# lukehollis/three-mlagents

Measured on NVIDIA B200. Metric: env_steps_per_sec, higher is better.
Workload: dtype f32+f64

## Files before the change

profiles/rollout_sass.py:

```python
from __future__ import annotations

import argparse
import os
import re
import subprocess
import sys
import tempfile

ROOT = os.path.dirname(os.path.dirname(os.path.abspath(__file__)))
FLAGS = ["-gencode", "arch=compute_100a,code=sm_100a", "-lineinfo", "-O3", "-std=c++17", "--expt-relaxed-constexpr"]
INS = re.compile(r"^\s+/\*([0-9a-f]{4,})\*/\s+(.*?)\s*;")


def _compile(tree, tmp):
    csrc = os.path.join(tree, "three-mlagents_b200", "csrc")
    cubin = os.path.join(tmp, "env_kernels.cubin")
    nvcc = os.path.join(os.environ.get("CUDA_HOME", "/usr/local/cuda"), "bin", "nvcc")
    r = subprocess.run([nvcc, *FLAGS, "-I", os.path.join(tree, "include"), "-Xptxas", "-v", "-cubin", "-o", cubin,
                        os.path.join(csrc, "env_kernels.cu")], capture_output=True, text=True)
    if r.returncode != 0:
        raise SystemExit(r.stdout + r.stderr)
    return cubin, r.stdout + r.stderr


def _ptxas(log, mangled):
    lines = log.splitlines()
    for n, line in enumerate(lines):
        if f"'{mangled}'" in line and "Compiling entry" in line:
            text = " ".join(lines[n + 1:n + 4])
            num = lambda pat: int(re.search(pat, text).group(1))
            return {"registers": num(r"Used (\d+) registers"), "stack_bytes": num(r"(\d+) bytes stack frame"),
                    "spill_store_bytes": num(r"(\d+) bytes spill stores"), "spill_load_bytes": num(r"(\d+) bytes spill loads")}
    raise SystemExit(f"{mangled}: no ptxas report")


def _sass(cubin, mangled):
    out = subprocess.run(["cuobjdump", "-sass", "-fun", mangled, cubin], capture_output=True, text=True, check=True).stdout
    return [(int(m.group(1), 16), m.group(2)) for m in map(INS.match, out.splitlines()) if m]


def _branch(ins):
    m = re.match(r"(@!?U?P\w+\s+)?BRA(\.U)?\s+(!?U?P\w+,\s*)?(0x[0-9a-f]+)", ins)
    if not m:
        return None
    return int(m.group(4), 16), bool(m.group(1) or m.group(3))


def _loops(code):
    loops = []
    for addr, ins in code:
        b = _branch(ins)
        if b and b[0] <= addr:
            loops.append((b[0], addr))
    return [(h, e) for h, e in loops if not any(h <= h2 and e2 <= e and (h2, e2) != (h, e) for h2, e2 in loops)]


def _shortest(code, head, end):
    body = [(a, ins) for a, ins in code if head <= a <= end]
    index = {a: n for n, (a, _) in enumerate(body)}
    inf = (1 << 30, 0, 0)
    best = [inf] * (len(body) + 1)
    best[0] = (0, 0, 0)
    for n, (a, ins) in enumerate(body):
        if best[n] == inf:
            continue
        c, br, st = best[n]
        here = (c + 1, br + (_branch(ins) is not None), st + ("STG" in ins and ".U8" in ins))
        if a == end:
            best[len(body)] = min(best[len(body)], here)
            continue
        b = _branch(ins)
        nxt = []
        if b is None or b[1]:
            if not re.match(r"(EXIT|RET)", ins):
                nxt.append(n + 1)
        if b and head < b[0] <= end and b[0] in index:
            nxt.append(index[b[0]])
        for m in nxt:
            best[m] = min(best[m], here)
    return best[len(body)]


def main():
    ap = argparse.ArgumentParser()
    ap.add_argument("--tree", default=ROOT, help="repository tree whose env_kernels.cu is compiled")
    ap.add_argument("--tasks", default="Ball3D,GridWorld,Push")
    args = ap.parse_args()
    with tempfile.TemporaryDirectory(prefix="rollout_sass_") as tmp:
        cubin, log = _compile(os.path.abspath(args.tree), tmp)
        for task in args.tasks.split(","):
            name = f"{task}Task"
            mangled = f"_Z19rollout_fast_kernelI{len(name)}{name}Ev7EnvPtrsjmmmiP6float4PiPfPh"
            res = _ptxas(log, mangled)
            code = _sass(cubin, mangled)
            print(f"rollout_fast_kernel<{name}>: {res['registers']} registers, stack {res['stack_bytes']} B, "
                  f"spills {res['spill_store_bytes']} B stored / {res['spill_load_bytes']} B loaded, {len(code) * 16} B of code")
            for head, end in _loops(code):
                ins, br, steps = _shortest(code, head, end)
                if not steps:
                    continue
                per = f", per step {ins / steps:.1f} instructions and {br / steps:.1f} branches"
                print(f"    loop 0x{head:x}-0x{end:x}: {end + 16 - head} B, shortest path {ins} instructions, "
                      f"{br} branches, {steps} steps{per}")


if __name__ == "__main__":
    sys.exit(main())
```

three-mlagents_b200/csrc/env_handle.cuh:

```cuda
#pragma once
#include "common.cuh"

struct tmla_env {
    int task;
    int64_t n;
    uint64_t seed, env_id_base, step_count;
    int device;
    void *buf[4];
    int *err_flag;
    void *d_stage, *h_stage;
    size_t stage_bytes;
    cudaStream_t own_stream;
    int32_t *d_ndone;
    int64_t rec_hint;
    cudaStream_t dev_stream;
    bool dev_dirty;
    cudaEvent_t dev_evt;
    int act_u8;
    void *shadow[4];
    int pend_seq;
    float2 *ep_log;
    int32_t ep_log_cap;
    int32_t *ep_log_count;
    void *rollout_plan;
    void (*rollout_plan_free)(void *);
};

struct DeviceGuard {
    int prev = -1;
    bool switched = false;
    explicit DeviceGuard(int dev) {
        if (cudaGetDevice(&prev) == cudaSuccess && prev != dev) switched = cudaSetDevice(dev) == cudaSuccess;
    }
    ~DeviceGuard() { if (switched) cudaSetDevice(prev); }
};
static inline void mark_device_path(tmla_env *h, cudaStream_t st) { h->dev_stream = st; h->dev_dirty = true; }
```

three-mlagents_b200/csrc/env_kernels.cu:

```cuda
#include <stdarg.h>
#include <stdlib.h>
#include <string.h>
#include <new>
#include <type_traits>
#if defined(__x86_64__)
#include <immintrin.h>
#endif
#include "envs.cuh"
#include "env_handle.cuh"

static int order_after_device_path(tmla_env *h) {
    if (!h->dev_dirty) return TMLA_OK;
    h->dev_dirty = false;
    cudaStreamCaptureStatus cap = cudaStreamCaptureStatusNone;
    if (cudaStreamIsCapturing(h->dev_stream, &cap) != cudaSuccess || cap != cudaStreamCaptureStatusNone ||
        cudaEventRecord(h->dev_evt, h->dev_stream) != cudaSuccess) {
        cudaGetLastError();
        TMLA_CUDA(cudaDeviceSynchronize());
        return TMLA_OK;
    }
    TMLA_CUDA(cudaStreamWaitEvent(h->own_stream, h->dev_evt, 0));
    return TMLA_OK;
}

struct EnvPtrs { void *buf[4]; };

static constexpr int kBlock = 128;

template <int D, int BLOCK, bool STREAMING>
__device__ __forceinline__ void block_store_obs(const float *s_obs, float *dst, int valid_envs) {
    const int total = valid_envs * D;
    if ((reinterpret_cast<uintptr_t>(dst) & 15u) == 0) {
        const int nvec = total >> 2;
        const float4 *s4 = reinterpret_cast<const float4 *>(s_obs);
        float4 *d4 = reinterpret_cast<float4 *>(dst);
        for (int v = threadIdx.x; v < nvec; v += BLOCK) {
            if (STREAMING) st_stream_f4(d4 + v, s4[v]);
            else d4[v] = s4[v];
        }
        for (int e = (nvec << 2) + threadIdx.x; e < total; e += BLOCK) dst[e] = s_obs[e];
    } else {
        for (int e = threadIdx.x; e < total; e += BLOCK) dst[e] = s_obs[e];
    }
}

template <int D>
__device__ __forceinline__ void thread_store_obs(const float *o, float *dst) {
#pragma unroll
    for (int j = 0; j < D; ++j) dst[j] = o[j];
}

template <class Task>
__global__ void __launch_bounds__(kBlock) reset_kernel(EnvPtrs p, int64_t n, uint64_t seed, uint64_t env_base,
                                                       uint64_t k, uint32_t tag, float *obs) {
    __shared__ __align__(16) float s_obs[kBlock * Task::D];
    const int64_t i0 = (int64_t)blockIdx.x * kBlock, i = i0 + threadIdx.x;
    if (i < n) {
        typename Task::State s;
        Task::reset(s, seed, env_base + (uint64_t)i, k, tag);
        Task::store(p.buf, i, s);
        float o[Task::D];
        Task::observe(s, o);
#pragma unroll
        for (int j = 0; j < Task::D; ++j) s_obs[threadIdx.x * Task::D + j] = o[j];
    }
    __syncthreads();
    if (obs) block_store_obs<Task::D, kBlock, false>(s_obs, obs + i0 * Task::D, (int)min((int64_t)kBlock, n - i0));
}

template <class Task>
__global__ void get_state_kernel(EnvPtrs p, int64_t n, typename Task::Wire *aos) {
    const int64_t i = (int64_t)blockIdx.x * blockDim.x + threadIdx.x;
    if (i < n) aos[i] = Task::to_wire(Task::load(p.buf, i));
}
template <class Task>
__global__ void set_state_kernel(EnvPtrs p, int64_t n, const typename Task::Wire *aos) {
    const int64_t i = (int64_t)blockIdx.x * blockDim.x + threadIdx.x;
    if (i < n) Task::store(p.buf, i, Task::from_wire(aos[i]));
}

template <class Task>
__global__ void __launch_bounds__(kBlock)
step_kernel(EnvPtrs p, int64_t n, uint64_t seed, uint64_t env_base, uint64_t step_index,
            const int32_t *__restrict__ actions, float *__restrict__ obs, float *__restrict__ reward,
            uint8_t *__restrict__ done, uint8_t *__restrict__ truncated, float *__restrict__ terminal_obs,
            float *__restrict__ ep_return, int32_t *__restrict__ ep_length, int32_t *n_done, int *err_flag,
            float *__restrict__ compact, int32_t *__restrict__ host_flags, int host_seq, int act_u8,
            const int32_t *ready, int32_t *dev_ready, int chunk_ctas, EnvPtrs shadow) {
    constexpr int D = Task::D;
    __shared__ __align__(16) float s_obs[kBlock * D];
    __shared__ __align__(16) float s_rew[kBlock];
    __shared__ __align__(16) uint8_t s_flag[2 * kBlock];
    const int64_t i0 = (int64_t)blockIdx.x * kBlock, i = i0 + threadIdx.x;
    if (ready) {
// ... 106 lines not shown
template <class Task>
__global__ void __launch_bounds__(kRollBlock)
rollout_random_kernel(EnvPtrs p, int64_t n, uint64_t seed, uint64_t env_base, uint64_t step0, int T,
                      float *__restrict__ obs_buf, int32_t *__restrict__ act_buf, float *__restrict__ rew_buf,
                      uint8_t *__restrict__ done_buf) {
    constexpr int D = Task::D, BLOCK = kRollBlock;
    constexpr bool STAGED = (D != 4);
    constexpr int NVEC = BLOCK * D / 4;
    __shared__ __align__(16) float s_obs[STAGED ? 2 * BLOCK * D : 4];
    const int64_t i0 = (int64_t)blockIdx.x * BLOCK, i = i0 + threadIdx.x;
    const bool active = i < n;
    const int valid = (int)min((int64_t)BLOCK, n - i0);
    const uint64_t env_id = env_base + (uint64_t)i;
    const int64_t row_floats = n * D;
    const bool vec_ok = obs_buf && valid == BLOCK && ((reinterpret_cast<uintptr_t>(obs_buf + i0 * D) & 15u) == 0) &&
                        ((row_floats & 3) == 0);
    const typename Task::Consts cst = Task::load_consts();
    typename Task::State s;
    TmlaActionStream as;
    if (active) {
        s = Task::load(p.buf, i);
        as.seek(seed, env_id, step0, Task::A);
    }
    float *orow = obs_buf ? obs_buf + i0 * D : nullptr;
    int64_t off = i;
    for (int t = 0; t < T; ++t) {
        const uint64_t k = step0 + (uint64_t)t;
        float *stage = STAGED ? s_obs + (t & 1) * BLOCK * D : s_obs;
        if (active) {
            float o[D];
            Task::observe(s, o);
            if (STAGED) stage_obs<D>(stage, o);
            else if (obs_buf) {
                float *dst = obs_buf + off * 4;
                if ((reinterpret_cast<uintptr_t>(obs_buf) & 15u) == 0) st_stream_f4(reinterpret_cast<float4 *>(dst), make_float4(o[0], o[1], o[2], o[3]));
                else { dst[0] = o[0]; dst[1] = o[1]; dst[2] = o[2]; dst[3] = o[3]; }
            }
            const int a = as.next(seed, env_id, step0, (uint32_t)t, Task::A);
            float r; bool term, trunc;
            Task::step(cst, s, a, r, term, trunc);
            s.ep_ret = __fadd_rn(s.ep_ret, r);
            const bool d = term || trunc;
            if (act_buf) __stcs(act_buf + off, a);
            if (rew_buf) __stcs(rew_buf + off, r);
            if (done_buf) __stcs(done_buf + off, (uint8_t)(d ? 1 : 0));
            if (d) Task::reset(s, seed, env_id, k + 1, TMLA_TAG_RESET);
        }
        if (STAGED) {
            __syncthreads();
            if (vec_ok) {
                const float4 *s4 = reinterpret_cast<const float4 *>(stage);
                float4 *d4 = reinterpret_cast<float4 *>(orow);
#pragma unroll
                for (int v = 0; v < (NVEC + BLOCK - 1) / BLOCK; ++v) {
                    const int e = v * BLOCK + threadIdx.x;
                    if ((v + 1) * BLOCK <= NVEC || e < NVEC) st_stream_f4(d4 + e, s4[e]);
                }
            } else if (obs_buf) {
                block_store_obs<D, BLOCK, true>(stage, orow, valid);
            }
            if (orow) orow += row_floats;
        }
        off += n;
    }
    if (active) Task::store(p.buf, i, s);
}

#ifndef TMLA_SPARE_EVERY
#define TMLA_SPARE_EVERY 64
#endif
static constexpr int kSpareEvery = TMLA_SPARE_EVERY;
#ifndef TMLA_ROLLOUT_UNROLL
#define TMLA_ROLLOUT_UNROLL 2
#endif
static constexpr int kRollUnroll = TMLA_ROLLOUT_UNROLL;
static_assert(kSpareEvery % 16 == 0 && ((kSpareEvery / 16) & (kSpareEvery / 16 - 1)) == 0, "a power-of-two number of action blocks");
static_assert(16 % kRollUnroll == 0, "the unrolled step loop covers whole action blocks");

template <class Task>
__device__ __noinline__ typename Task::Spare draw_spare(uint64_t seed, uint64_t env_id, uint32_t episode) {
    return Task::draw(seed, env_id, episode, TMLA_TAG_RESET);
}

template <class Task>
__global__ void __launch_bounds__(kRollBlock)
rollout_fast_kernel(EnvPtrs p, uint32_t n, uint64_t seed, uint64_t env_base, uint64_t step0, int T,
                    float4 *__restrict__ obs4, int32_t *__restrict__ act_buf, float *__restrict__ rew_buf,
                    uint8_t *__restrict__ done_buf) {
    constexpr int D = Task::D, BLOCK = kRollBlock, NVEC = BLOCK * D / 4;
    static_assert(Task::A <= 16, "actions are packed as 4-bit digits");
    constexpr bool DIRECT = (D == 6);
    constexpr bool STAGED = (D != 4) && !DIRECT;
    static_assert((BLOCK * D) % 4 == 0, "block rows must be whole float4s");
    __shared__ __align__(16) float s_stage[STAGED ? 2 * BLOCK * D : 4];
    const uint32_t tid = threadIdx.x, i = blockIdx.x * BLOCK + tid;
    const uint64_t env_id = env_base + (uint64_t)i;
    const typename Task::Consts cst = Task::load_consts();
    typename Task::State s = Task::load(p.buf, i);
    float *orow = reinterpret_cast<float *>(obs4) + (size_t)i * D;
    float4 *vrow = obs4 + blockIdx.x * NVEC + tid;
    int32_t *arow = act_buf + i;
    float *rrow = rew_buf + i;
    uint8_t *drow = done_buf + i;
    const uint32_t rowfloats = n * D;
    uint32_t sb = 0;
    [[maybe_unused]] typename Task::Spare sp;
    [[maybe_unused]] bool have_spare = false;
    auto step = [&](uint64_t digits, uint32_t j, uint64_t kb) {
        float o[D];
        Task::observe(s, o);
        if constexpr (STAGED) {
            if constexpr (D % 2 == 0) {
                float2 *s2 = reinterpret_cast<float2 *>(s_stage + sb + tid * D);
#pragma unroll
                for (int q = 0; q < D / 2; ++q) s2[q] = make_float2(o[2 * q], o[2 * q + 1]);
            } else {
#pragma unroll
                for (int q = 0; q < D; ++q) s_stage[sb + tid * D + q] = o[q];
            }
        } else if constexpr (DIRECT) {
            float2 *d2 = reinterpret_cast<float2 *>(orow);
#pragma unroll
            for (int q = 0; q < D / 2; ++q) __stcs(d2 + q, make_float2(o[2 * q], o[2 * q + 1]));
        } else {
            st_stream_f4(reinterpret_cast<float4 *>(orow), make_float4(o[0], o[1], o[2], o[3]));
        }
        const int a = (int)((uint32_t)(digits >> (4 * j)) & 15u);
        float r; bool term, trunc;
        Task::step(cst, s, a, r, term, trunc);
        s.ep_ret = __fadd_rn(s.ep_ret, r);
        const bool d = term || trunc;
        __stcs(arow, a);
        __stcs(rrow, r);
        __stcs(drow, (uint8_t)(d ? 1 : 0));
        if (d) {
            if constexpr (Task::HAS_SPARE) {
                const uint32_t e = Task::next_episode(s);
                if (!have_spare) sp = draw_spare<Task>(seed, env_id, e);
                Task::begin_episode(s, sp, e);
                have_spare = false;
            } else {
                Task::reset(s, seed, env_id, kb + j + 1, TMLA_TAG_RESET);
            }
        }
        if constexpr (STAGED) {
            if constexpr (BLOCK == 32) __syncwarp(); else __syncthreads();
            const float4 *s4 = reinterpret_cast<const float4 *>(s_stage + sb);
#pragma unroll
            for (int v = 0; v < (NVEC + BLOCK - 1) / BLOCK; ++v) {
                const int e = v * BLOCK + tid;
                if ((v + 1) * BLOCK <= NVEC || e < NVEC) st_stream_f4(vrow + v * BLOCK, s4[e]);
            }
            sb ^= BLOCK * D;
            vrow += rowfloats / 4;
        } else {
            orow += rowfloats;
        }
        arow += n; rrow += n; drow += n;
    };
    uint64_t kb = step0 & ~(uint64_t)15;
    uint32_t j = (uint32_t)step0 & 15u;
    uint32_t left = (uint32_t)T;
    for (uint32_t nb = 0; left != 0; ++nb, kb += 16, j = 0) {
        const uint64_t digits = TmlaActionStream::block_digits(seed, env_id, kb >> 4, Task::A);
        if constexpr (Task::HAS_SPARE) {
            if ((nb & (kSpareEvery / 16 - 1)) == 0 && !have_spare) {
                sp = Task::draw(seed, env_id, Task::next_episode(s), TMLA_TAG_RESET);
                have_spare = true;
            }
        }
        if (j == 0 && left >= 16) {
#pragma unroll kRollUnroll
            for (uint32_t q = 0; q < 16; ++q) step(digits, q, kb);
            left -= 16;
        } else {
            const uint32_t je = min(16u, j + left);
            left -= je - j;
#pragma unroll 1
            for (; j < je; ++j) step(digits, j, kb);
        }
    }
    Task::store(p.buf, i, s);
}

template <int A>
__device__ __forceinline__ void categorical(const float *l, bool deterministic, float u, int &action, float &logp) {
    float m = l[0];
#pragma unroll
    for (int j = 1; j < A; ++j) m = fmaxf(m, l[j]);
    float e[A], sum = 0.0f;
#pragma unroll
    for (int j = 0; j < A; ++j) { e[j] = expf(l[j] - m); sum += e[j]; }
    int a = 0;
    if (deterministic) {
#pragma unroll
        for (int j = 1; j < A; ++j) if (l[j] > l[a]) a = j;
    } else {
        const float target = u * sum;
        float c = 0.0f;
        a = A - 1;
        bool found = false;
#pragma unroll
        for (int j = 0; j < A; ++j) {
            c += e[j];
            if (!found && target < c) { a = j; found = true; }
        }
    }
    action = a;
    logp = (l[a] - m) - logf(sum);
}

template <class Task>
__global__ void __launch_bounds__(kBlock)
step_policy_kernel(EnvPtrs p, int64_t n, uint64_t seed, uint64_t env_base, uint64_t step_index,
                   const uint64_t *__restrict__ step_base, const float *__restrict__ logits, int deterministic,
                   int64_t row_index, float *__restrict__ obs_next, int32_t *__restrict__ act, float *__restrict__ logp_out,
                   float *__restrict__ rew, uint8_t *__restrict__ done, int32_t *trunc_count,
                   int32_t *__restrict__ trunc_index, float *__restrict__ trunc_obs, int32_t trunc_capacity,
                   float *ep_stats, float2 *__restrict__ ep_log, int32_t ep_log_cap, int32_t *ep_log_count) {
    constexpr int D = Task::D, A = Task::A;
    __shared__ __align__(16) float s_obs[kBlock * D];
    __shared__ float s_ep[3];
    const int64_t i0 = (int64_t)blockIdx.x * kBlock, i = i0 + threadIdx.x;
    const uint64_t k = step_base ? (*step_base + (uint64_t)row_index) : step_index;
    const unsigned lane = threadIdx.x & 31u, lanes_below = (1u << lane) - 1u;
    if (threadIdx.x < 3) s_ep[threadIdx.x] = 0.0f;
    __syncthreads();
    const bool live = i < n;
    const uint64_t env_id = env_base + (uint64_t)i;
    typename Task::State s;
    float o[D];
    bool d = false, trunc_only = false;
    float ep_r = 0.0f, ep_l = 0.0f;
    if (live) {
        const typename Task::Consts cst = Task::load_consts();
        s = Task::load(p.buf, i);
        float l[A];
#pragma unroll
        for (int j = 0; j < A; ++j) l[j] = logits[i * A + j];
        float u = 0.0f;
        if (!deterministic) u = tmla_u24(tmla_stream_block(seed, env_id, k, TMLA_TAG_SAMPLE, 0).x);
        int a; float lp;
        categorical<A>(l, deterministic != 0, u, a, lp);
        float r; bool term, trunc;
        Task::step(cst, s, a, r, term, trunc);
        s.ep_ret = __fadd_rn(s.ep_ret, r);
        d = term || trunc;
        trunc_only = trunc && !term;
        if (act) act[i] = a;
        if (logp_out) logp_out[i] = lp;
        rew[i] = r;
        done[i] = d ? 1 : 0;
        Task::observe(s, o);
        if (d) { ep_r = s.ep_ret; ep_l = (float)s.steps; }
    }
    if (trunc_count) {
        const unsigned m = __ballot_sync(0xffffffffu, trunc_only);
        if (m) {
            const int leader = __ffs(m) - 1;
            int base = 0;
            if ((int)lane == leader) base = atomicAdd(trunc_count, __popc(m));
            base = __shfl_sync(0xffffffffu, base, leader);
            if (trunc_only) {
                const int slot = base + __popc(m & lanes_below);
                if (slot < trunc_capacity) {
// ... 128 lines not shown
    }
    uint64_t t[4]; uint8_t m8[32];
    _mm256_storeu_si256((__m256i *)t, acc); _mm256_storeu_si256((__m256i *)m8, vmx);
    const uint64_t o = t[0] | t[1] | t[2] | t[3];
    *ored |= (o | (o >> 32)) & 0xFFFFFFFFull;
    for (int k = 0; k < 32; ++k) *mx = m8[k] > *mx ? m8[k] : *mx;
    return i;
}
__attribute__((target("avx2"))) static int64_t stage_actions64_avx2(const int64_t *src, uint8_t *dst, int64_t n, uint64_t *ored, uint32_t *mx) {
    __m256i acc = _mm256_setzero_si256(), vmx = _mm256_setzero_si256();
    const __m256i lo = _mm256_setr_epi32(0, 2, 4, 6, 0, 2, 4, 6), perm = _mm256_setr_epi32(0, 4, 1, 5, 2, 6, 3, 7);
    int64_t i = 0;
    for (; i + 32 <= n; i += 32) {
        __m256i w[4];
        for (int k = 0; k < 4; ++k) {
            const __m256i x = _mm256_loadu_si256((const __m256i *)(src + i + 8 * k)), y = _mm256_loadu_si256((const __m256i *)(src + i + 8 * k + 4));
            acc = _mm256_or_si256(acc, _mm256_or_si256(x, y));
            const __m256i xl = _mm256_permutevar8x32_epi32(x, lo), yl = _mm256_permutevar8x32_epi32(y, lo);
            w[k] = _mm256_inserti128_si256(xl, _mm256_castsi256_si128(yl), 1);
        }
        __m256i p = _mm256_packus_epi16(_mm256_packs_epi32(w[0], w[1]), _mm256_packs_epi32(w[2], w[3]));
        p = _mm256_permutevar8x32_epi32(p, perm);
        vmx = _mm256_max_epu8(vmx, p);
        _mm256_storeu_si256((__m256i *)(dst + i), p);
    }
    uint64_t t[4]; uint8_t m8[32];
    _mm256_storeu_si256((__m256i *)t, acc); _mm256_storeu_si256((__m256i *)m8, vmx);
    const uint64_t o = t[0] | t[1] | t[2] | t[3];
    *ored |= (o & ~7ull) ? 0xFFFFFFFFull : (o & 7ull);
    for (int k = 0; k < 32; ++k) *mx = m8[k] > *mx ? m8[k] : *mx;
    return i;
}
#endif

extern "C" {

int tmla_task_from_name(const char *name) {
    if (!name) { tmla_set_error("task name is NULL"); return TMLA_EINVAL; }
    if (!strcmp(name, "basic")) return TMLA_BASIC;
    if (!strcmp(name, "ball3d")) return TMLA_BALL3D;
    if (!strcmp(name, "gridworld")) return TMLA_GRIDWORLD;
    if (!strcmp(name, "push")) return TMLA_PUSH;
    if (!strcmp(name, "walljump")) return TMLA_WALLJUMP;
    if (!strcmp(name, "brickbreak")) return TMLA_BRICKBREAK;
    if (!strcmp(name, "bicycle")) return TMLA_BICYCLE;
    if (!strcmp(name, "glider")) return TMLA_GLIDER;
    tmla_set_error("no CUDA backend for task '%s' (have: basic, ball3d, gridworld, push, walljump, brickbreak, bicycle, glider)", name);
    return TMLA_EINVAL;
}
#define TASK_META(fn, table)                                                                   \
    int fn(int task) {                                                                         \
        if (task < 0 || task >= TMLA_NUM_TASKS) { tmla_set_error(#fn ": unknown task %d", task); return TMLA_EINVAL; } \
        return table[task];                                                                    \
    }
TASK_META(tmla_task_obs_dim, kObsDim)
TASK_META(tmla_task_num_actions, kNumActions)
TASK_META(tmla_task_max_steps, kMaxSteps)
TASK_META(tmla_task_state_size, kStateSize)

int tmla_create(int task, int64_t n_envs, uint64_t seed, uint64_t env_id_base, int device, tmla_env **out) {
    TMLA_REQUIRE(out != nullptr, "out is NULL");
    TMLA_REQUIRE(task >= 0 && task < TMLA_NUM_TASKS, "unknown task");
    TMLA_REQUIRE(n_envs > 0 && n_envs < (int64_t)1 << 31, "n_envs must be in (0, 2^31)");
    int ndev = 0;
    TMLA_CUDA(cudaGetDeviceCount(&ndev));
    TMLA_REQUIRE(device >= 0 && device < ndev, "no such CUDA device (this library has no CPU path)");
    DeviceGuard guard(device);
    tmla_env *h = new (std::nothrow) tmla_env();
    if (!h) { tmla_set_error("out of host memory"); return TMLA_ENOMEM; }
    memset(h, 0, sizeof(*h));
    h->task = task; h->n = n_envs; h->seed = seed; h->env_id_base = env_id_base; h->device = device;
    h->rec_hint = 256;
    int nbuf = 0;
    size_t pb[4] = {0, 0, 0, 0};
    TASK_SWITCH(task, nbuf = TaskT::NBUF; for (int b = 0; b < nbuf; ++b) pb[b] = TaskT::plane_bytes(b));
    for (int b = 0; b < nbuf; ++b) {
        cudaError_t e = cudaMalloc(&h->buf[b], pb[b] * (size_t)n_envs);
        if (e != cudaSuccess) { tmla_set_error("cudaMalloc(state plane %d): %s", b, cudaGetErrorString(e)); tmla_destroy(h); return TMLA_ENOMEM; }
    }
    const int D = kObsDim[task];
    h->stage_bytes = stage_layout(n_envs, D).end + 64;
    if (cudaMalloc(&h->d_stage, h->stage_bytes) != cudaSuccess || cudaMallocHost(&h->h_stage, h->stage_bytes) != cudaSuccess ||
        cudaMalloc((void **)&h->err_flag, sizeof(int)) != cudaSuccess || cudaMalloc((void **)&h->d_ndone, sizeof(int32_t)) != cudaSuccess ||
        cudaStreamCreateWithFlags(&h->own_stream, cudaStreamNonBlocking) != cudaSuccess ||
        cudaEventCreateWithFlags(&h->dev_evt, cudaEventDisableTiming) != cudaSuccess) {
        tmla_set_error("allocating staging buffers: %s", cudaGetErrorString(cudaGetLastError()));
        tmla_destroy(h);
        return TMLA_ENOMEM;
    }
    TMLA_CUDA(cudaMemset(h->err_flag, 0, sizeof(int)));
    memset((char *)h->h_stage + stage_layout(n_envs, D).end, 0, 64);
    TMLA_CUDA(cudaMemset((char *)h->d_stage + stage_layout(n_envs, D).flags, 0, 16));
    TMLA_CUDA(cudaMemset((char *)h->d_stage + stage_layout(n_envs, D).end, 0, 64));
    TMLA_CUDA(cudaMemset(h->d_ndone, 0, sizeof(int32_t)));
    *out = h;
    int rc = tmla_reset(h, nullptr, nullptr);
    if (rc) return rc;
    TMLA_CUDA(cudaStreamSynchronize(nullptr));
    h->dev_dirty = false;
    return TMLA_OK;
}

int tmla_destroy(tmla_env *h) {
    if (!h) return TMLA_OK;
    DeviceGuard guard(h->device);
    for (int b = 0; b < 4; ++b) if (h->buf[b]) cudaFree(h->buf[b]);
    if (h->d_stage) cudaFree(h->d_stage);
    if (h->h_stage) cudaFreeHost(h->h_stage);
    if (h->err_flag) cudaFree(h->err_flag);
    if (h->d_ndone) cudaFree(h->d_ndone);
    for (int b = 0; b < 4; ++b) if (h->shadow[b]) cudaFree(h->shadow[b]);
    if (h->own_stream) cudaStreamDestroy(h->own_stream);
    if (h->dev_evt) cudaEventDestroy(h->dev_evt);
    if (h->rollout_plan && h->rollout_plan_free) h->rollout_plan_free(h->rollout_plan);
    delete h;
    return TMLA_OK;
}

int tmla_seed(tmla_env *h, uint64_t seed) { TMLA_REQUIRE(h, "handle is NULL"); h->seed = seed; return TMLA_OK; }
int64_t tmla_num_envs(const tmla_env *h) { return h ? h->n : 0; }
uint64_t tmla_step_count(const tmla_env *h) { return h ? h->step_count : 0; }
int tmla_advance_steps(tmla_env *h, uint64_t n) { TMLA_REQUIRE(h, "handle is NULL"); h->step_count += n; return TMLA_OK; }

int tmla_reset(tmla_env *h, float *obs, void *stream) {
    TMLA_REQUIRE(h, "handle is NULL");
    DeviceGuard guard(h->device);
    cudaStream_t st = (cudaStream_t)stream;
    if (st != h->own_stream) mark_device_path(h, st);
    TASK_SWITCH(h->task, (reset_kernel<TaskT><<<grid_for(h->n), kBlock, 0, st>>>(
                             ptrs_of(h), h->n, h->seed, h->env_id_base, h->step_count, TMLA_TAG_RESET_ALL, obs)));
    TMLA_LAUNCH_CHECK();
    return TMLA_OK;
}

int tmla_step(tmla_env *h, const int32_t *actions, float *obs, float *reward, uint8_t *done, uint8_t *truncated,
              float *terminal_obs, float *ep_return, int32_t *ep_length, void *stream) {
    TMLA_REQUIRE(h, "handle is NULL");
    TMLA_REQUIRE(actions && obs && reward && done && truncated, "actions/obs/reward/done/truncated must be non-NULL");
    DeviceGuard guard(h->device);
    cudaStream_t st = (cudaStream_t)stream;
    mark_device_path(h, st);
    TASK_SWITCH(h->task, (step_kernel<TaskT><<<grid_for(h->n), kBlock, 0, st>>>(
                             ptrs_of(h), h->n, h->seed, h->env_id_base, h->step_count, actions, obs, reward, done,
                             truncated, terminal_obs, ep_return, ep_length, nullptr, h->err_flag, nullptr, nullptr, 0, 0, nullptr, nullptr, 1, EnvPtrs{})));
    TMLA_LAUNCH_CHECK();
    h->step_count += 1;
    return TMLA_OK;
}

static bool host_step_mapped() {
    static const bool mapped = [] { const char *e = getenv("TMLA_HOST_STEP"); return !(e && !strcmp(e, "copy")); }();
    return mapped;
}
static int wait_block_published(tmla_env *h, const char *block, int seq, int64_t *n_done) {
    const StageLayout L = stage_layout(h->n, kObsDim[h->task]);
    const int32_t *bflags = (const int32_t *)(block + (L.flags - L.obs));
    volatile const int32_t *hseq = (volatile const int32_t *)bflags + 2;
    cudaStream_t st = h->own_stream;
    static const bool poll = [] { const char *e = getenv("TMLA_HOST_STEP"); return !(e && !strcmp(e, "sync")); }();
    if (!poll) TMLA_CUDA(cudaStreamSynchronize(st));
    for (uint32_t spins = 1; *hseq != seq; ++spins) {
        if ((spins & 4095u) == 0) {
            const cudaError_t q = cudaStreamQuery(st);
            if (q != cudaErrorNotReady) { TMLA_CUDA(q); if (*hseq != seq) { tmla_set_error("step kernel finished without publishing its results"); return TMLA_ECUDA; } }
        }
    }
    __sync_synchronize();
    if (n_done) *n_done = bflags[0];
    if (bflags[1]) {
        tmla_set_error("an action outside [0,%d) was passed to step()", kNumActions[h->task]);
        return TMLA_EACTION;
    }
    return TMLA_OK;
}
static int step_into_block(tmla_env *h, char *block, int64_t *n_done) {
    DeviceGuard guard(h->device);
    { const int rc = order_after_device_path(h); if (rc) return rc; }
    const int act_u8 = h->act_u8;
    h->act_u8 = 0;
    const int64_t n = h->n;
    const int D = kObsDim[h->task];
    const StageLayout L = stage_layout(n, D);
    char *d = (char *)h->d_stage, *p = (char *)h->h_stage;
    cudaStream_t st = h->own_stream;
    int32_t *dflags = (int32_t *)(d + L.flags);
    const int32_t *bflags = (const int32_t *)(block + (L.flags - L.obs));
    if (host_step_mapped()) {
        char *b = block - L.obs;
        const int seq = (int)((h->step_count + 1) & 0x3FFFFFFF) | 0x40000000;
        volatile int32_t *hseq = (volatile int32_t *)(b + L.flags) + 2;
        *hseq = 0;
        TASK_SWITCH(h->task, (step_kernel<TaskT><<<grid_for(n), kBlock, 0, st>>>(
                                 ptrs_of(h), n, h->seed, h->env_id_base, h->step_count, (const int32_t *)(p + L.act),
// ... 235 lines not shown
    TMLA_REQUIRE(h && records && floats_per_record, "NULL argument");
    const StageLayout L = stage_layout(h->n, kObsDim[h->task]);
    *records = (const float *)((char *)h->h_stage + L.crec);
    *floats_per_record = record_words(kObsDim[h->task]);
    return TMLA_OK;
}

int tmla_step_host(tmla_env *h, const int32_t *actions, float *obs, float *reward, uint8_t *done, uint8_t *truncated,
                   float *terminal_obs, float *ep_return, int32_t *ep_length, int64_t *n_done) {
    TMLA_REQUIRE(h, "handle is NULL");
    TMLA_REQUIRE(actions && obs && reward && done && truncated, "actions/obs/reward/done/truncated must be non-NULL");
    const int64_t n = h->n;
    const int D = kObsDim[h->task];
    const StageLayout L = stage_layout(n, D);
    char *p = (char *)h->h_stage;
    { const int rc = tmla_stage_actions(h, actions, 4); if (rc) return rc; }
    int64_t nd = 0;
    const int rc = step_into_block(h, p + L.obs, &nd);
    if (rc != TMLA_OK && rc != TMLA_EACTION) return rc;
    memcpy(obs, p + L.obs, 4 * n * D);
    memcpy(reward, p + L.rew, 4 * n);
    memcpy(done, p + L.done, n);
    memcpy(truncated, p + L.trunc, n);
    const size_t rec = (size_t)4 * record_words(D);
    for (int64_t s = 0; s < nd; ++s) {
        const float *r = (const float *)(p + L.crec + rec * s);
        int32_t i, l;
        memcpy(&i, r, 4); memcpy(&l, r + 2, 4);
        if (terminal_obs) memcpy(terminal_obs + (size_t)i * D, r + 3, (size_t)4 * D);
        if (ep_return) ep_return[i] = r[1];
        if (ep_length) ep_length[i] = l;
    }
    if (n_done) *n_done = nd;
    return rc;
}

int tmla_reset_host(tmla_env *h, float *obs) {
    TMLA_REQUIRE(h && obs, "handle/obs is NULL");
    DeviceGuard guard(h->device);
    { const int rc = order_after_device_path(h); if (rc) return rc; }
    const size_t bytes = (size_t)4 * h->n * kObsDim[h->task];
    const StageLayout L = stage_layout(h->n, kObsDim[h->task]);
    char *d = (char *)h->d_stage, *p = (char *)h->h_stage;
    int rc = tmla_reset(h, (float *)(d + L.obs), h->own_stream);
    if (rc) return rc;
    TMLA_CUDA(cudaMemcpyAsync(p + L.obs, d + L.obs, bytes, cudaMemcpyDeviceToHost, h->own_stream));
    TMLA_CUDA(cudaStreamSynchronize(h->own_stream));
    if (obs != (float *)(p + L.obs)) memcpy(obs, p + L.obs, bytes);
    return TMLA_OK;
}

int tmla_get_state(tmla_env *h, void *aos, void *stream) {
    TMLA_REQUIRE(h && aos, "handle/aos is NULL");
    DeviceGuard guard(h->device);
    mark_device_path(h, (cudaStream_t)stream);
    TASK_SWITCH(h->task, (get_state_kernel<TaskT><<<grid_for(h->n), kBlock, 0, (cudaStream_t)stream>>>(
                             ptrs_of(h), h->n, (typename TaskT::Wire *)aos)));
    TMLA_LAUNCH_CHECK();
    return TMLA_OK;
}
int tmla_set_state(tmla_env *h, const void *aos, void *stream) {
    TMLA_REQUIRE(h && aos, "handle/aos is NULL");
    DeviceGuard guard(h->device);
    mark_device_path(h, (cudaStream_t)stream);
    TASK_SWITCH(h->task, (set_state_kernel<TaskT><<<grid_for(h->n), kBlock, 0, (cudaStream_t)stream>>>(
                             ptrs_of(h), h->n, (const typename TaskT::Wire *)aos)));
    TMLA_LAUNCH_CHECK();
    return TMLA_OK;
}
int tmla_check_actions(tmla_env *h, void *stream) {
    TMLA_REQUIRE(h, "handle is NULL");
    DeviceGuard guard(h->device);
    int err = 0;
    TMLA_CUDA(cudaMemcpyAsync(&err, h->err_flag, sizeof(int), cudaMemcpyDeviceToHost, (cudaStream_t)stream));
    TMLA_CUDA(cudaStreamSynchronize((cudaStream_t)stream));
    if (err) {
        TMLA_CUDA(cudaMemsetAsync(h->err_flag, 0, sizeof(int), (cudaStream_t)stream));
        tmla_set_error("an action outside [0,%d) was passed to step()", kNumActions[h->task]);
        return TMLA_EACTION;
    }
    return TMLA_OK;
}

int tmla_rollout_random(tmla_env *h, int T, float *obs_buf, int32_t *act_buf, float *rew_buf, uint8_t *done_buf, void *stream) {
    TMLA_REQUIRE(h, "handle is NULL");
    TMLA_REQUIRE(T > 0, "T must be positive");
    DeviceGuard guard(h->device);
    mark_device_path(h, (cudaStream_t)stream);
    const int D = kObsDim[h->task];
    const bool fast = obs_buf && act_buf && rew_buf && done_buf && (h->n % kRollBlock == 0) &&
                      ((reinterpret_cast<uintptr_t>(obs_buf) & 15u) == 0) && ((int64_t)T * h->n * D / 4 < ((int64_t)1 << 31));
    const unsigned grid = (unsigned)ceil_div64(h->n, kRollBlock);
    if (fast) {
        TASK_SWITCH(h->task, (rollout_fast_kernel<TaskT><<<grid, kRollBlock, 0, (cudaStream_t)stream>>>(
                                 ptrs_of(h), (uint32_t)h->n, h->seed, h->env_id_base, h->step_count, T,
                                 reinterpret_cast<float4 *>(obs_buf), act_buf, rew_buf, done_buf)));
    } else {
        TASK_SWITCH(h->task, (rollout_random_kernel<TaskT><<<grid, kRollBlock, 0, (cudaStream_t)stream>>>(
                                 ptrs_of(h), h->n, h->seed, h->env_id_base, h->step_count, T, obs_buf, act_buf, rew_buf, done_buf)));
    }
    TMLA_LAUNCH_CHECK();
    h->step_count += (uint64_t)T;
    return TMLA_OK;
}

int tmla_step_policy(tmla_env *h, const float *logits, int deterministic, int32_t row_index, float *obs_next,
                     int32_t *act, float *logp, float *rew, uint8_t *done, int32_t *trunc_count, int32_t *trunc_index,
                     float *trunc_obs, int32_t trunc_capacity, float *ep_stats, const uint64_t *step_base, void *stream) {
    TMLA_REQUIRE(h, "handle is NULL");
    TMLA_REQUIRE(logits && obs_next && rew && done, "logits/obs_next/rew/done must be non-NULL");
    TMLA_REQUIRE(!trunc_count || (trunc_index && trunc_obs && trunc_capacity > 0), "truncation list is incomplete");
    DeviceGuard guard(h->device);
    mark_device_path(h, (cudaStream_t)stream);
    TASK_SWITCH(h->task, (step_policy_kernel<TaskT><<<grid_for(h->n), kBlock, 0, (cudaStream_t)stream>>>(
                             ptrs_of(h), h->n, h->seed, h->env_id_base, h->step_count, step_base, logits, deterministic,
                             (int64_t)row_index, obs_next, act, logp, rew, done, trunc_count, trunc_index, trunc_obs,
                             trunc_capacity, ep_stats, h->ep_log, h->ep_log_cap, h->ep_log_count)));
    TMLA_LAUNCH_CHECK();
    if (!step_base) h->step_count += 1;
    return TMLA_OK;
}

int tmla_selftest_arith(uint64_t *out3, void *stream) {
    TMLA_REQUIRE(out3, "out3 is NULL");
    TMLA_CUDA(cudaMemsetAsync(out3, 0, 3 * sizeof(uint64_t), (cudaStream_t)stream));
    selftest_arith_kernel<<<148 * 8, 256, 0, (cudaStream_t)stream>>>((unsigned long long *)out3);
    TMLA_LAUNCH_CHECK();
    return TMLA_OK;
}

int tmla_counter_add(uint64_t *counter, uint64_t n, void *stream) {
    TMLA_REQUIRE(counter, "counter is NULL");
    counter_add_kernel<<<1, 1, 0, (cudaStream_t)stream>>>(counter, n);
    TMLA_LAUNCH_CHECK();
    return TMLA_OK;
}

}
```

Before: 151.1 billion.

## Chain back-to-back rollout launches with programmatic dependent launch and a per-slice ring

Consecutive rollout_fast_kernel launches on the same stream now use programmatic stream serialization. Each block takes a dynamic slice through an atomic counter, then waits on a generation-tagged ring entry published by the block of the previous launch that finished that slice. A block can start as soon as its own slice is ready rather than after the whole previous grid has drained, which is meant to hide launch gaps and tail idle time. The cost is extra atomics, a spin-wait with nanosleep, a device memory ring and more complex ordering. A clock-instrumentation build and profiling script are added alongside.

```diff
diff --git a/profiles/rollout_clocks.py b/profiles/rollout_clocks.py
--- /dev/null
+++ b/profiles/rollout_clocks.py
@@ -0,0 +1,137 @@
+from __future__ import annotations
+
+import argparse
+import ctypes as C
+import json
+import os
+import shutil
+import statistics
+import subprocess
+import sys
+import tempfile
+
+import numpy as np
+
+ROOT = os.path.dirname(os.path.dirname(os.path.abspath(__file__)))
+N, T = 65536, 128
+
+
+def _build(tmp):
+    pkg = os.path.join(tmp, "three-mlagents_b200")
+    shutil.copytree(os.path.join(ROOT, "three-mlagents_b200"), pkg, ignore=shutil.ignore_patterns("lib", "__pycache__"))
+    shutil.copytree(os.path.join(ROOT, "include"), os.path.join(tmp, "include"))
+    env = dict(os.environ, TMLA_EXTRA_NVCC_FLAGS="-DTMLA_ROLLOUT_CLOCKS")
+    out = subprocess.run([sys.executable, os.path.join(pkg, "build.py"), "--force"], env=env, capture_output=True, text=True)
+    if out.returncode != 0:
+        raise SystemExit(out.stdout + out.stderr)
+    return out.stdout.strip().splitlines()[-1]
+
+
+def _stats(x):
+    x = np.asarray(x, dtype=np.float64)
+    return {"median": float(np.median(x)), "min": float(x.min()), "max": float(x.max())}
+
+
+def _measure(launches, torch, CudaVecEnv, lib):
+    env = CudaVecEnv("ball3d", N, seed=1)
+    obs = torch.empty((T, N, 6), device="cuda")
+    act = torch.empty((T, N), dtype=torch.int32, device="cuda")
+    rew = torch.empty((T, N), device="cuda")
+    done = torch.empty((T, N), dtype=torch.uint8, device="cuda")
+    for _ in range(20):
+        env.rollout_random(T, obs, act, rew, done)
+    torch.cuda.synchronize()
+    lib.tmla_debug_rollout_clocks(None, 0, 1)
+    e0, e1 = torch.cuda.Event(enable_timing=True), torch.cuda.Event(enable_timing=True)
+    e0.record()
+    for _ in range(launches):
+        env.rollout_random(T, obs, act, rew, done)
+    e1.record()
+    torch.cuda.synchronize()
+    event_us = e0.elapsed_time(e1) / launches * 1e3
+    grid = N // 32
+    buf = (C.c_ulonglong * (4 * grid * launches))()
+    got = lib.tmla_debug_rollout_clocks(buf, grid * launches, 1)
+    env.close()
+    if got != grid * launches:
+        raise SystemExit(f"{got} warp records, expected {grid * launches}")
+    rec = np.frombuffer(buf, dtype=np.uint64).reshape(-1, 4)
+    entry, first, exit_ = (rec[:, k].astype(np.int64) for k in range(3))
+    sm, sched, launch = (rec[:, 3] & 0xFF).astype(np.int64), ((rec[:, 3] >> 8) & 3).astype(np.int64), (rec[:, 3] >> 32).astype(np.int64)
+    t0 = entry.min()
+    entry, first, exit_ = entry - t0, first - t0, exit_ - t0
+    ids = sorted(set(launch.tolist()))
+    spans, gaps, prologue, idle, tail = [], [], [], [], []
+    frac = {3: [], 4: [], "other": []}
+    bounds = []
+    for L in ids:
+        m = launch == L
+        a, b = int(entry[m].min()), int(exit_[m].max())
+        bounds.append((a, b))
+        spans.append((b - a) / 1e3)
+        prologue.extend(((first[m] - entry[m]) / 1e3).tolist())
+        key = sm[m] * 4 + sched[m]
+        uniq, inv, cnt = np.unique(key, return_inverse=True, return_counts=True)
+        per = cnt[inv]
+        f = (exit_[m] - a) / (b - a)
+        for g in (3, 4):
+            frac[g].extend(f[per == g].tolist())
+        frac["other"].extend(f[(per != 3) & (per != 4)].tolist())
+        last = np.zeros(len(uniq), dtype=np.int64)
+        np.maximum.at(last, inv, exit_[m])
+        idle.append(float(np.mean((b - last) / (b - a))))
+        tail.append(float(np.mean(cnt)))
+    for k in range(1, len(bounds)):
+        gaps.append((bounds[k][0] - bounds[k - 1][1]) / 1e3)
+    ts = np.unique(np.concatenate([entry, first, exit_]))
+    span_med = statistics.median(spans)
+    return {
+        "event_us_per_launch": event_us,
+        "span_us": _stats(spans),
+        "gap_us": _stats(gaps),
+        "prologue_us": _stats(prologue),
+        "exit_fraction_by_warps_per_scheduler": {str(g): {**_stats(v), "warps": len(v)} for g, v in frac.items() if v},
+        "scheduler_idle_fraction_mean": float(np.mean(idle)),
+        "warps_per_busy_scheduler_mean": float(np.mean(tail)),
+        "launch_period_us": (bounds[-1][0] - bounds[0][0]) / 1e3 / (len(bounds) - 1),
+        "idle_plus_gap_fraction": float(np.mean(idle)) + max(statistics.median(gaps), 0.0) / span_med,
+        "globaltimer_resolution_ns": int(np.diff(ts).min()) if len(ts) > 1 else None,
+    }
+
+
+def main():
+    ap = argparse.ArgumentParser()
+    ap.add_argument("--launches", type=int, default=50)
+    ap.add_argument("--out", default=os.path.join(ROOT, "profiles", "rollout_clocks_1gpu.json"))
+    args = ap.parse_args()
+    q = "name,power.limit,clocks.max.sm"
+    card = subprocess.run(["nvidia-smi", f"--query-gpu={q}", "--format=csv,noheader", "-i", "0"],
+                          capture_output=True, text=True, check=True).stdout.strip()
+    result = {"card": dict(zip(q.split(","), [c.strip() for c in card.split(",")])),
+              "shape": f"ball3d {N} envs x {T} steps, {args.launches} back-to-back launches"}
+    tmp = tempfile.mkdtemp(prefix="rollout_clocks_")
+    try:
+        os.environ["TMLA_LIB"] = _build(tmp)
+        sys.path.insert(0, ROOT)
+        import torch
+
+        from three_mlagents_b200 import native
+        from three_mlagents_b200.vec_env import CudaVecEnv
+
+        lib = native.lib
+        lib.tmla_debug_rollout_clocks.restype = C.c_int
+        lib.tmla_debug_rollout_clocks.argtypes = [C.c_void_p, C.c_int64, C.c_int]
+        for mode, flag in (("unchained", "0"), ("chained", "1")):
+            os.environ["TMLA_ROLLOUT_CHAIN"] = flag
+            result[mode] = _measure(args.launches, torch, CudaVecEnv, lib)
+            print(mode, json.dumps(result[mode]), file=sys.stderr, flush=True)
+    finally:
+        shutil.rmtree(tmp, ignore_errors=True)
+    os.makedirs(os.path.dirname(os.path.abspath(args.out)), exist_ok=True)
+    with open(args.out, "w") as f:
+        json.dump(result, f, indent=1)
+    print(json.dumps(result))
+
+
+if __name__ == "__main__":
+    main()
diff --git a/profiles/rollout_sass.py b/profiles/rollout_sass.py
--- a/profiles/rollout_sass.py
+++ b/profiles/rollout_sass.py
@@ -90,7 +90,8 @@
         cubin, log = _compile(os.path.abspath(args.tree), tmp)
         for task in args.tasks.split(","):
             name = f"{task}Task"
-            mangled = f"_Z19rollout_fast_kernelI{len(name)}{name}Ev7EnvPtrsjmmmiP6float4PiPfPh"
+            prefix = f"_Z19rollout_fast_kernelI{len(name)}{name}E"
+            mangled = re.search(rf"Compiling entry function '({prefix}\w*)'", log).group(1)
             res = _ptxas(log, mangled)
             code = _sass(cubin, mangled)
             print(f"rollout_fast_kernel<{name}>: {res['registers']} registers, stack {res['stack_bytes']} B, "
diff --git a/three-mlagents_b200/csrc/env_handle.cuh b/three-mlagents_b200/csrc/env_handle.cuh
--- a/three-mlagents_b200/csrc/env_handle.cuh
+++ b/three-mlagents_b200/csrc/env_handle.cuh
@@ -22,6 +22,9 @@
     float2 *ep_log;
     int32_t ep_log_cap;
     int32_t *ep_log_count;
+    void *roll_ring;
+    uint32_t roll_gen;
+    bool roll_chain;
     void *rollout_plan;
     void (*rollout_plan_free)(void *);
 };
@@ -34,4 +37,5 @@
     }
     ~DeviceGuard() { if (switched) cudaSetDevice(prev); }
 };
-static inline void mark_device_path(tmla_env *h, cudaStream_t st) { h->dev_stream = st; h->dev_dirty = true; }
+static inline void mark_device_path(tmla_env *h, cudaStream_t st) { h->dev_stream = st; h->dev_dirty = true; h->roll_chain = false; }
+static inline size_t roll_ring_bytes(int64_t n) { return 16 + 2 * sizeof(uint64_t) * (size_t)ceil_div64(n, 32); }
diff --git a/three-mlagents_b200/csrc/env_kernels.cu b/three-mlagents_b200/csrc/env_kernels.cu
--- a/three-mlagents_b200/csrc/env_kernels.cu
+++ b/three-mlagents_b200/csrc/env_kernels.cu
@@ -10,6 +10,7 @@
 #include "env_handle.cuh"
 
 static int order_after_device_path(tmla_env *h) {
+    h->roll_chain = false;
     if (!h->dev_dirty) return TMLA_OK;
     h->dev_dirty = false;
     cudaStreamCaptureStatus cap = cudaStreamCaptureStatusNone;
@@ -282,23 +283,87 @@
     return Task::draw(seed, env_id, episode, TMLA_TAG_RESET);
 }
 
+#ifdef TMLA_ROLLOUT_CLOCKS
+static constexpr uint32_t kRollClockCap = 1u << 18;
+__device__ unsigned long long g_roll_clocks[4 * kRollClockCap];
+__device__ unsigned int g_roll_clock_n;
+__device__ __forceinline__ unsigned long long globaltimer() {
+    unsigned long long t;
+    asm volatile("mov.u64 %0, %%globaltimer;" : "=l"(t));
+    return t;
+}
+#endif
+
+struct RollChain {
+    uint32_t *count;
+    unsigned long long *ring;
+    uint32_t gen;
+    int chained;
+};
+
+__device__ __forceinline__ uint32_t ld_relaxed_gpu(const uint32_t *p) {
+    uint32_t v;
+    asm volatile("ld.relaxed.gpu.global.u32 %0, [%1];" : "=r"(v) : "l"(p) : "memory");
+    return v;
+}
+__device__ __forceinline__ unsigned long long ld_acquire_gpu(const unsigned long long *p) {
+    unsigned long long v;
+    asm volatile("ld.acquire.gpu.global.u64 %0, [%1];" : "=l"(v) : "l"(p) : "memory");
+    return v;
+}
+__device__ __forceinline__ void st_release_gpu(unsigned long long *p, unsigned long long v) {
+    asm volatile("st.release.gpu.global.u64 [%0], %1;" ::"l"(p), "l"(v) : "memory");
+}
+
+__device__ __forceinline__ uint32_t roll_take_slice(const RollChain c) {
+    const uint32_t grid = gridDim.x, par = c.gen & 1u, base = (c.gen >> 1) * grid;
+    const uint32_t t = atomicAdd(c.count + par, 1u) - base;
+    if (!c.chained) return t;
+    const uint32_t pbase = ((c.gen - 1u) >> 1) * grid;
+    if (ld_relaxed_gpu(c.count + 2 + (par ^ 1u)) - pbase >= grid) asm volatile("griddepcontrol.wait;" ::: "memory");
+    const unsigned long long *slot = c.ring + (size_t)(par ^ 1u) * grid + t;
+    const uint32_t want = c.gen;
+    unsigned long long v;
+    for (uint32_t ns = 32; (uint32_t)((v = ld_acquire_gpu(slot)) >> 32) != want; ns = ns < 1024 ? 2 * ns : ns) __nanosleep(ns);
+    return (uint32_t)v;
+}
+
+__device__ __forceinline__ void roll_publish(const RollChain c, uint32_t slice) {
+    const uint32_t grid = gridDim.x, par = c.gen & 1u, base = (c.gen >> 1) * grid;
+    const uint32_t pos = atomicAdd(c.count + 2 + par, 1u) - base;
+    st_release_gpu(c.ring + (size_t)par * grid + pos, ((unsigned long long)(c.gen + 1u) << 32) | slice);
+    if (c.chained) asm volatile("griddepcontrol.wait;" ::: "memory");
+}
+
 template <class Task>
 __global__ void __launch_bounds__(kRollBlock)
 rollout_fast_kernel(EnvPtrs p, uint32_t n, uint64_t seed, uint64_t env_base, uint64_t step0, int T,
                     float4 *__restrict__ obs4, int32_t *__restrict__ act_buf, float *__restrict__ rew_buf,
-                    uint8_t *__restrict__ done_buf) {
+                    uint8_t *__restrict__ done_buf, const RollChain chain) {
     constexpr int D = Task::D, BLOCK = kRollBlock, NVEC = BLOCK * D / 4;
     static_assert(Task::A <= 16, "actions are packed as 4-bit digits");
     constexpr bool DIRECT = (D == 6);
     constexpr bool STAGED = (D != 4) && !DIRECT;
     static_assert((BLOCK * D) % 4 == 0, "block rows must be whole float4s");
     __shared__ __align__(16) float s_stage[STAGED ? 2 * BLOCK * D : 4];
-    const uint32_t tid = threadIdx.x, i = blockIdx.x * BLOCK + tid;
+#ifdef TMLA_ROLLOUT_CLOCKS
+    const unsigned long long ck_entry = globaltimer();
+    unsigned long long ck_first = 0;
+#endif
+    const uint32_t tid = threadIdx.x;
+    uint32_t slice = blockIdx.x;
+    if (chain.count) {
+        if (tid == 0) slice = roll_take_slice(chain);
+        slice = __shfl_sync(0xffffffffu, slice, 0);
+        __syncwarp();
+        asm volatile("griddepcontrol.launch_dependents;" ::: "memory");
+    }
+    const uint32_t i = slice * BLOCK + tid;
     const uint64_t env_id = env_base + (uint64_t)i;
     const typename Task::Consts cst = Task::load_consts();
     typename Task::State s = Task::load(p.buf, i);
     float *orow = reinterpret_cast<float *>(obs4) + (size_t)i * D;
-    float4 *vrow = obs4 + blockIdx.x * NVEC + tid;
+    float4 *vrow = obs4 + slice * NVEC + tid;
     int32_t *arow = act_buf + i;
     float *rrow = rew_buf + i;
     uint8_t *drow = done_buf + i;
@@ -369,6 +434,9 @@
                 have_spare = true;
             }
         }
+#ifdef TMLA_ROLLOUT_CLOCKS
+        if (nb == 0) ck_first = globaltimer();
+#endif
         if (j == 0 && left >= 16) {
 #pragma unroll kRollUnroll
             for (uint32_t q = 0; q < 16; ++q) step(digits, q, kb);
@@ -381,6 +449,26 @@
         }
     }
     Task::store(p.buf, i, s);
+    if (chain.count) {
+        __threadfence();
+        __syncwarp();
+        if (tid == 0) roll_publish(chain, slice);
+    }
+#ifdef TMLA_ROLLOUT_CLOCKS
+    if (tid == 0) {
+        const unsigned long long ck_exit = globaltimer();
+        uint32_t smid, warpid;
+        asm volatile("mov.u32 %0, %%smid;" : "=r"(smid));
+        asm volatile("mov.u32 %0, %%warpid;" : "=r"(warpid));
+        const uint32_t r = atomicAdd(&g_roll_clock_n, 1u);
+        if (r < kRollClockCap) {
+            unsigned long long *rec = g_roll_clocks + 4 * (size_t)r;
+            rec[0] = ck_entry; rec[1] = ck_first; rec[2] = ck_exit;
+            const uint32_t launch = chain.count ? chain.gen : r / gridDim.x;
+            rec[3] = smid | ((warpid & 3u) << 8) | ((unsigned long long)launch << 32);
+        }
+    }
+#endif
 }
 
 template <int A>
@@ -675,6 +763,7 @@
     h->stage_bytes = stage_layout(n_envs, D).end + 64;
     if (cudaMalloc(&h->d_stage, h->stage_bytes) != cudaSuccess || cudaMallocHost(&h->h_stage, h->stage_bytes) != cudaSuccess ||
         cudaMalloc((void **)&h->err_flag, sizeof(int)) != cudaSuccess || cudaMalloc((void **)&h->d_ndone, sizeof(int32_t)) != cudaSuccess ||
+        cudaMalloc(&h->roll_ring, roll_ring_bytes(n_envs)) != cudaSuccess ||
         cudaStreamCreateWithFlags(&h->own_stream, cudaStreamNonBlocking) != cudaSuccess ||
         cudaEventCreateWithFlags(&h->dev_evt, cudaEventDisableTiming) != cudaSuccess) {
         tmla_set_error("allocating staging buffers: %s", cudaGetErrorString(cudaGetLastError()));
@@ -686,6 +775,7 @@
     TMLA_CUDA(cudaMemset((char *)h->d_stage + stage_layout(n_envs, D).flags, 0, 16));
     TMLA_CUDA(cudaMemset((char *)h->d_stage + stage_layout(n_envs, D).end, 0, 64));
     TMLA_CUDA(cudaMemset(h->d_ndone, 0, sizeof(int32_t)));
+    TMLA_CUDA(cudaMemsetAsync(h->roll_ring, 0, roll_ring_bytes(n_envs), nullptr));
     *out = h;
     int rc = tmla_reset(h, nullptr, nullptr);
     if (rc) return rc;
@@ -702,6 +792,7 @@
     if (h->h_stage) cudaFreeHost(h->h_stage);
     if (h->err_flag) cudaFree(h->err_flag);
     if (h->d_ndone) cudaFree(h->d_ndone);
+    if (h->roll_ring) cudaFree(h->roll_ring);
     for (int b = 0; b < 4; ++b) if (h->shadow[b]) cudaFree(h->shadow[b]);
     if (h->own_stream) cudaStreamDestroy(h->own_stream);
     if (h->dev_evt) cudaEventDestroy(h->dev_evt);
@@ -1103,19 +1194,47 @@
     return TMLA_OK;
 }
 
+static bool rollout_chain_enabled() {
+    const char *e = getenv("TMLA_ROLLOUT_CHAIN");
+    return !(e && !strcmp(e, "0"));
+}
+
 int tmla_rollout_random(tmla_env *h, int T, float *obs_buf, int32_t *act_buf, float *rew_buf, uint8_t *done_buf, void *stream) {
     TMLA_REQUIRE(h, "handle is NULL");
     TMLA_REQUIRE(T > 0, "T must be positive");
     DeviceGuard guard(h->device);
-    mark_device_path(h, (cudaStream_t)stream);
+    cudaStream_t st = (cudaStream_t)stream;
+    const bool after_fast = h->roll_chain && h->dev_stream == st;
+    mark_device_path(h, st);
     const int D = kObsDim[h->task];
     const bool fast = obs_buf && act_buf && rew_buf && done_buf && (h->n % kRollBlock == 0) &&
                       ((reinterpret_cast<uintptr_t>(obs_buf) & 15u) == 0) && ((int64_t)T * h->n * D / 4 < ((int64_t)1 << 31));
     const unsigned grid = (unsigned)ceil_div64(h->n, kRollBlock);
     if (fast) {
-        TASK_SWITCH(h->task, (rollout_fast_kernel<TaskT><<<grid, kRollBlock, 0, (cudaStream_t)stream>>>(
-                                 ptrs_of(h), (uint32_t)h->n, h->seed, h->env_id_base, h->step_count, T,
-                                 reinterpret_cast<float4 *>(obs_buf), act_buf, rew_buf, done_buf)));
+        cudaStreamCaptureStatus cap = cudaStreamCaptureStatusNone;
+        if (cudaStreamIsCapturing(st, &cap) != cudaSuccess) { cudaGetLastError(); cap = cudaStreamCaptureStatusActive; }
+        RollChain chain{};
+        if (rollout_chain_enabled() && cap == cudaStreamCaptureStatusNone) {
+            if (h->roll_gen >= 0x80000000u) {
+                TMLA_CUDA(cudaMemsetAsync(h->roll_ring, 0, roll_ring_bytes(h->n), st));
+                h->roll_gen = 0;
+            }
+            chain.count = (uint32_t *)h->roll_ring;
+            chain.ring = (unsigned long long *)((char *)h->roll_ring + 16);
+            chain.gen = h->roll_gen;
+            chain.chained = after_fast && h->roll_gen > 0;
+        }
+        cudaLaunchConfig_t cfg;
+        memset(&cfg, 0, sizeof(cfg));
+        cfg.gridDim = dim3(grid); cfg.blockDim = dim3(kRollBlock); cfg.stream = st;
+        cudaLaunchAttribute attr;
+        attr.id = cudaLaunchAttributeProgrammaticStreamSerialization;
+        attr.val.programmaticStreamSerializationAllowed = 1;
+        cfg.attrs = &attr; cfg.numAttrs = chain.chained ? 1 : 0;
+        TASK_SWITCH(h->task, TMLA_CUDA(cudaLaunchKernelEx(&cfg, rollout_fast_kernel<TaskT>, ptrs_of(h), (uint32_t)h->n, h->seed,
+                                                          h->env_id_base, h->step_count, T, reinterpret_cast<float4 *>(obs_buf),
+                                                          act_buf, rew_buf, done_buf, chain)));
+        if (chain.count) { h->roll_gen += 1; h->roll_chain = true; }
     } else {
         TASK_SWITCH(h->task, (rollout_random_kernel<TaskT><<<grid, kRollBlock, 0, (cudaStream_t)stream>>>(
                                  ptrs_of(h), h->n, h->seed, h->env_id_base, h->step_count, T, obs_buf, act_buf, rew_buf, done_buf)));
@@ -1150,6 +1269,17 @@
     return TMLA_OK;
 }
 
+#ifdef TMLA_ROLLOUT_CLOCKS
+int tmla_debug_rollout_clocks(unsigned long long *out, int64_t cap, int reset) {
+    unsigned int n = 0;
+    TMLA_CUDA(cudaMemcpyFromSymbol(&n, g_roll_clock_n, sizeof(n)));
+    if (n > kRollClockCap) n = kRollClockCap;
+    if (out && cap > 0) TMLA_CUDA(cudaMemcpyFromSymbol(out, g_roll_clocks, 4 * sizeof(unsigned long long) * (size_t)(cap < n ? cap : n)));
+    if (reset) { const unsigned int z = 0; TMLA_CUDA(cudaMemcpyToSymbol(g_roll_clock_n, &z, sizeof(z))); }
+    return (int)n;
+}
+#endif
+
 int tmla_counter_add(uint64_t *counter, uint64_t n, void *stream) {
     TMLA_REQUIRE(counter, "counter is NULL");
     counter_add_kernel<<<1, 1, 0, (cudaStream_t)stream>>>(counter, n);
```

New measurement: 156.2 billion, median of 6. +3.4%, better.
